# keras-team/keras-rs

Measured on AMD Instinct MI355X. Metric: embedding lookups/sec + DCN fwd+bwd step time, 26-table DLRM batch 65 536, higher is better.
Workload: dtype bf16; 1 GPU; C3 DLRM-small: 26 tables x 1000000 rows x 128 (bf16), global batch 65536, multi-hot ml_perf lengths (sum L = 214), uniform ids, DotInteraction(F=27) + 3 x FeatureCross(d=3456, projection=512), fused Adagrad on tables; global_batch=65536, parallelism=single GPU

## Files before the change

### include/krs.h

```cpp
#ifndef KRS_H_
#define KRS_H_

#include <stddef.h>
#include <stdint.h>

#ifdef __cplusplus
extern "C" {
#endif

#define KRS_VERSION 100

typedef enum krs_status {
  KRS_OK = 0,
  KRS_ERR_INVALID = -1,
  KRS_ERR_UNSUPPORTED = -2,
  KRS_ERR_LAUNCH = -3,
  KRS_ERR_WORKSPACE = -4
} krs_status;

typedef enum krs_dtype { KRS_F32 = 0, KRS_BF16 = 1, KRS_I8 = 2 } krs_dtype;
typedef enum krs_itype { KRS_I32 = 0, KRS_I64 = 1 } krs_itype;

typedef enum krs_combiner { KRS_SUM = 0, KRS_MEAN = 1, KRS_SQRTN = 2 } krs_combiner;

// ... 159 lines not shown
             void* workspace, size_t workspace_bytes, void* stream);
size_t krs_gemm_workspace_bytes(int64_t m, int64_t n, int64_t k, int a_is_km);

size_t krs_gemm_cross_bwd_workspace_bytes(int64_t m, int64_t n);
int krs_gemm_cross_bwd(const void* a, int64_t lda, const void* bt, int64_t ldb,
                       const void* r, int64_t ldr, float beta,
                       void* g_out, int64_t ldg,
                       const void* x0, const void* u, void* dz, void* dx0, int64_t ld, int dx0_accumulate,
                       const void* u_upper, int fold_direct, float* dbias, int64_t m, int64_t n, int64_t k, int act, int dtype,
                       void* workspace, size_t workspace_bytes, void* stream);
int krs_gemm_dense_bwd(const void* a, int64_t lda, const void* bt, int64_t ldb, void* g_out, int64_t ldg,
                       const void* y, void* dz, int64_t ld, float* dbias, int64_t m, int64_t n, int64_t k, int act,
                       int dtype, void* workspace, size_t workspace_bytes, void* stream);
enum { KRS_CROSS_BWD_NONE = 0, KRS_CROSS_BWD_TWO_CALL = 1, KRS_CROSS_BWD_PP64 = 2, KRS_CROSS_BWD_PP256 = 3 };
int krs_gemm_cross_bwd_last_route(int* epilogue);
int krs_gemm_cross_bwd_plan_route(const void* a, int64_t lda, const void* bt, int64_t ldb, const void* r, int64_t ldr,
                                  float beta, void* g_out, int64_t ldg, const void* x0, const void* u, void* dz, void* dx0,
                                  int64_t ld, int dx0_accumulate, const void* u_upper, int64_t m, int64_t n, int64_t k,
                                  int dtype, int* epilogue);

enum {
  KRS_GEMM_KERNEL_NONE = 0, KRS_GEMM_KERNEL_GENERIC = 1, KRS_GEMM_KERNEL_MFMA = 2, KRS_GEMM_KERNEL_GLDS = 3,
  KRS_GEMM_KERNEL_TN_GLDS = 4, KRS_GEMM_KERNEL_PP256 = 5, KRS_GEMM_KERNEL_PP256_KSTRIDED = 6, KRS_GEMM_KERNEL_PP64 = 7,
  KRS_GEMM_KERNEL_THIN = 8, KRS_GEMM_KERNEL_ROWDOT = 9, KRS_GEMM_KERNEL_SMALLK = 10
};
enum { KRS_GEMM_REDUCE_NONE = 0, KRS_GEMM_REDUCE_SCALAR = 1, KRS_GEMM_REDUCE_VEC4 = 2, KRS_GEMM_REDUCE_VEC8 = 3 };
typedef struct krs_gemm_route {
  int32_t kernel;
  int32_t splits;
  int32_t reduce;
  int32_t epilogue;
  int32_t ep_vec;
  int32_t thin_width;
  int32_t thin_is_a;
  int32_t schedule;
} krs_gemm_route;
enum { KRS_GEMM_SCHED_LDS_LANDING = 1, KRS_GEMM_SCHED_STAGGER = 2, KRS_GEMM_SCHED_X_IS_X0 = 4 };
int krs_gemm_last_route(krs_gemm_route* route);
int krs_gemm_plan_route(const void* a, int64_t lda, int a_is_km, const void* b, int64_t ldb, int b_is_nk, const void* c,
                        int64_t ldc, int64_t m, int64_t n, int64_t k, int in_dtype, int out_dtype,
                        const krs_gemm_epilogue* epilogue, size_t workspace_bytes, krs_gemm_route* route);

enum { KRS_GEMM_OPT_PIPELINE = 0, KRS_GEMM_OPT_EPI_SCHEDULE = 1 };
int krs_gemm_set_option(int key, int value);

enum { KRS_EMBED_OPT_PLAN = 2, KRS_EMBED_OPT_HOTROWS = 3, KRS_EMBED_OPT_RANK = 4, KRS_EMBED_OPT_APPLY_DEPTH = 5 };
int krs_embed_set_option(int key, int value);

size_t krs_colsum_workspace_bytes(int64_t m, int64_t n);
int krs_cross_epilogue_fwd(const void* u, const void* x0, const void* x, void* y,
                           int64_t m, int64_t n, int64_t ld, float diag_scale,
                           int dtype, void* stream);
// ... 237 lines not shown
```

### keras_rs_amd/_lib.py

```python

from __future__ import annotations

import ctypes as C
import os

import numpy as np
import torch

_HERE = os.path.dirname(os.path.abspath(__file__))
LIB_PATH = os.environ.get("KRS_LIB", os.path.join(_HERE, "libkrs_hip.so"))

F32, BF16, I8 = 0, 1, 2
I32, I64 = 0, 1
SUM, MEAN, SQRTN = 0, 1, 2
COMBINERS = {"sum": SUM, "mean": MEAN, "sqrtn": SQRTN}
ACT_NONE, ACT_RELU, ACT_SIGMOID, ACT_TANH = 0, 1, 2, 3
FLAG_ID_OUT_OF_RANGE = 1
FLAG_BAD_OFFSETS = 2
FLAG_CAPACITY_OVERFLOW = 4
FLAG_NONFINITE_ROW = 8
MAX_LIST = 4096

TABLE_DT = np.dtype(
    [("weights", "<u8"), ("slot", "<u8"), ("row_base", "<i8"), ("vocab", "<i4"), ("lr", "<f4")]
# ... 17 lines not shown
        ("ldx", C.c_int64),
        ("u_out", C.c_void_p),
        ("ldu", C.c_int64),
        ("r", C.c_void_p),
        ("ldr", C.c_int64),
        ("beta", C.c_float),
    ]


class GemmRoute(C.Structure):
    _fields_ = [(name, C.c_int32) for name in
                ("kernel", "splits", "reduce", "epilogue", "ep_vec", "thin_width", "thin_is_a", "schedule")]


GEMM_OPT_PIPELINE, GEMM_OPT_EPI_SCHEDULE = 0, 1
GEMM_SCHED_LDS_LANDING, GEMM_SCHED_STAGGER, GEMM_SCHED_X_IS_X0 = 1, 2, 4


class GemmQ8Route(C.Structure):
    _fields_ = [(name, C.c_int32) for name in ("kernel", "ep_vec", "k_tail", "epilogue")]


class EmbedFwdRoute(C.Structure):
    _fields_ = [(name, C.c_int32) for name in
                ("kernel", "lpr", "has_w", "stream", "hot_rows", "bpg", "table_dtype", "out_dtype")] + [("blocks", C.c_int64)]


class DotRoute(C.Structure):
    _fields_ = [(name, C.c_int32) for name in
                ("kernel", "dtype", "ks", "fr", "self", "multi", "acc", "ng", "lps_log2", "spw", "launches",
                 "lds_bytes")] + [("blocks", C.c_int64)]
# ... 18 lines not shown
    "krs_embed_bag_bwd_fused_sgd": (_I, _EMBED_BWD + [_P, _P]),
    "krs_embed_bag_bwd_fused_adagrad": (_I, _EMBED_BWD + [_P, _P]),
    "krs_embed_bag_bwd_fused_adagrad_rowwise": (_I, _EMBED_BWD + [_P, _P]),
    "krs_embed_bag_bwd_fused_adam": (_I, _EMBED_BWD + [_F, _F, _F, _F, _P, _P]),
    "krs_embed_bag_bwd_fused_ftrl": (_I, _EMBED_BWD + [_F, _F, _F, _F, _P, _P]),
    "krs_embed_bag_bwd_fused_adam_dyn": (_I, _EMBED_BWD + [_F, _F, _F, _P, _P, _P]),
    "krs_store_f32": (_I, [_P, _I64, _P, _I, _P]),
    "krs_embed_bag_bwd_sparse": (_I, [_P, _I, _P, _P, _P, _I, _I64, _I, _I, _I64, _P, _P, _P, _P, _P]),
    "krs_gemm": (_I, [_P, _I64, _I, _P, _I64, _I, _P, _I64, _I64, _I64, _I64, _I, _I, _P, _P, _SZ, _P]),
    "krs_gemm_workspace_bytes": (_SZ, [_I64, _I64, _I64, _I]),
    "krs_gemm_cross_bwd_workspace_bytes": (_SZ, [_I64, _I64]),
    "krs_gemm_cross_bwd": (_I, [_P, _I64, _P, _I64, _P, _I64, _F, _P, _I64, _P, _P, _P, _P, _I64, _I, _P, _I, _P,
                                _I64, _I64, _I64, _I, _I, _P, _SZ, _P]),
    "krs_gemm_dense_bwd": (_I, [_P, _I64, _P, _I64, _P, _I64, _P, _P, _I64, _P, _I64, _I64, _I64, _I, _I, _P, _SZ, _P]),
    "krs_gemm_cross_bwd_last_route": (_I, [_P]),
    "krs_gemm_cross_bwd_plan_route": (_I, [_P, _I64, _P, _I64, _P, _I64, _F, _P, _I64, _P, _P, _P, _P, _I64, _I, _P, _I64,
                                           _I64, _I64, _I, _P]),
    "krs_gemm_last_route": (_I, [_P]),
    "krs_gemm_plan_route": (_I, [_P, _I64, _I, _P, _I64, _I, _P, _I64, _I64, _I64, _I64, _I, _I, _P, _SZ, _P]),
    "krs_gemm_set_option": (_I, [_I, _I]),
    "krs_embed_set_option": (_I, [_I, _I]),
    "krs_colsum_workspace_bytes": (_SZ, [_I64, _I64]),
    "krs_cross_epilogue_fwd": (_I, [_P, _P, _P, _P, _I64, _I64, _I64, _F, _I, _P]),
    "krs_cross_epilogue_bwd": (_I, [_P, _P, _P, _P, _P, _P, _I, _P, _P, _I64, _I64, _I64, _F, _I, _I, _P, _SZ, _P]),
    "krs_cast_transpose": (_I, [_P, _I64, _I64, _I64, _I, _P, _I64, _P, _I64, _I, _P]),
    "krs_cast_transpose_many": (_I, [_I, _P, _P, _P, _I, _P, _P, _I, _P]),
    "krs_dense_act_bwd": (_I, [_P, _I64, _P, _I64, _P, _I64, _P, _I64, _I64, _I, _I, _P, _SZ, _P]),
    "krs_dense_adagrad": (_I, [_P, _P, _P, _P, _I, _F, _F, _P]),
    "krs_colsum": (_I, [_P, _I64, _I64, _I64, _I, _P, _P, _SZ, _P]),
    "krs_dot_interaction_fwd": (_I, [_P, _P, _I, _I64, _I, _I, _I, _I, _P, _I64, _P]),
# ... 162 lines not shown
```

### keras_rs_amd/csrc/gemm.hip

```cpp
#include <algorithm>
#include <cstdlib>
#include <cstring>

#include "gemm_device.h"
#include "gemm_plan.h"
#include "gemm_ring64.h"

namespace krs {
namespace {

constexpr int BM = gplan::kTile, BN = gplan::kTile;
constexpr int ROW_BYTES = gplan::kRowBytes;
constexpr int TILE_BYTES = gplan::kTileBytes;

template <int ES>
__device__ __forceinline__ void load_kstrided(const char* base, int64_t ld, int64_t row0, int64_t k0,
                                              int64_t rows, int64_t kk, u32x4 (&r)[4]) {
  constexpr int RPB = 16 / ES;
  constexpr int NRB = BM / RPB;
  const int t = threadIdx.x;
  const int rb = t % NRB;
  const int kb = t / NRB;
  const int64_t row = row0 + rb * RPB;
#pragma unroll
// ... 50 lines not shown
                                                          int64_t wm0, int64_t wn0, int split, EpiOperands (&o)[4],
                                                          const float* pre_bias = nullptr) {
  static_assert(NPFC == 2 || NPFC == 4, "two or four chunks of operands are fetched ahead");
  if constexpr (PREBIAS && NPFC == 4) {
#pragma unroll
    for (int c = 0; c < 4; ++c) epi_settle<EPI == 1>(o[c]);
  }
  epi_process<EPI, PREBIAS>(p, acc[0][0], o[0], stage, wm0, wn0, split, pre_bias);
  if constexpr (NPFC == 2) epi_prefetch<EPI>(p, o[2], wm0 + 64, wn0);
  epi_process<EPI, PREBIAS>(p, acc[0][1], o[1], stage, wm0 + 32, wn0, split, pre_bias);
  if constexpr (NPFC == 2) epi_prefetch<EPI>(p, o[3], wm0 + 96, wn0);
  epi_process<EPI, PREBIAS>(p, acc[1][0], o[2], stage, wm0 + 64, wn0, split, pre_bias);
  epi_process<EPI, PREBIAS>(p, acc[1][1], o[3], stage, wm0 + 96, wn0, split, pre_bias);
}

__device__ __forceinline__ void epi_land_issue(const GemmParams& p, uint32_t land, int64_t row0, int64_t wn0) {
  const int lane = threadIdx.x & 63;
  const int64_t gnc = min(wn0 + (lane & 7) * 8, p.n - 8);
  const uint16_t* src[8];
#pragma unroll
  for (int it = 0; it < 4; ++it) {
    const int64_t gmc = min(row0 + it * 8 + (lane >> 3), p.m - 1);
    src[it] = reinterpret_cast<const uint16_t*>(p.ep.x) + gmc * p.ep.ldx + gnc;
    src[4 + it] = reinterpret_cast<const uint16_t*>(p.ep.x0) + gmc * p.ep.ldx + gnc;
  }
#pragma unroll
  for (int i = 0; i < 8; ++i) {
    uint32_t keep;
    asm volatile("s_mov_b32 %0, m0\n\ts_mov_b32 m0, %2\n\ts_nop 0\n\tglobal_load_lds_dwordx4 %1, off nt\n\ts_mov_b32 m0, %0"
                 : "=&s"(keep)
                 : "v"(src[i]), "s"(land + i * 1024)
                 : "memory");
  }
}
template <int BEHIND>
__device__ __forceinline__ void epi_land_read(const char* land, EpiOperands& o) {
  static_assert(BEHIND >= 8 && BEHIND < 64, "vmcnt is a 6-bit counter");
  asm volatile("s_waitcnt vmcnt(%0)" ::"n"(BEHIND) : "memory");
  const int lane = threadIdx.x & 63;
#pragma unroll
  for (int it = 0; it < 4; ++it) {
    o.ex[it] = *reinterpret_cast<const uint4*>(land + it * 1024 + lane * 16);
    o.ex0[it] = *reinterpret_cast<const uint4*>(land + 4096 + it * 1024 + lane * 16);
  }
}
__device__ __forceinline__ void gemm_epilogue_wave128_land(const GemmParams& p, f32x16 (&acc)[2][2][2], float* stage, char* land,
                                                           int64_t wm0, int64_t wn0, int split, EpiOperands (&o)[4],
                                                           const float* pre_bias) {
// ... 385 lines not shown
        dz[q] = gx0 * act_grad_from_output(p.f_act, uv[q]);
        db[q] += dz[q];
        const float told = DX0 == 1 ? tv[q] : (DX0 == 2 ? rv[q] * tv[q] : 0.0f);
        tv[q] = __builtin_fmaf(g[q], uv[q], told);
        if (p.f_fold) tv[q] += g[q];
      }
      store8_bf16_nt(p.f_dz, gm * p.f_ld + gn, dz);
      if constexpr (DX0 != 3) store8_bf16_nt(p.f_dx0, gm * p.f_ld + gn, tv);
    }
    __builtin_amdgcn_fence(__ATOMIC_ACQ_REL, "wavefront");
    if (c < 3) {
      ld_x0u(c + 1, (c + 1) & 1);
      ld_rd(c + 1, (c + 1) & 1);
    }
  }
  if (p.f_partial) {
#pragma unroll
    for (int q = 0; q < 8; ++q) {
      float t = db[q];
      t += __shfl_xor(t, 8);
      t += __shfl_xor(t, 16);
      t += __shfl_xor(t, 32);
      db[q] = t;
    }
    if ((lane >> 3) == 0 && gn < p.n) {
      float* dst = p.f_partial + group * p.n + gn;
      *reinterpret_cast<float4*>(dst) = make_float4(db[0], db[1], db[2], db[3]);
      *reinterpret_cast<float4*>(dst + 4) = make_float4(db[4], db[5], db[6], db[7]);
    }
  }
// ... 255 lines not shown
  }
  if constexpr (NPFC > 0)
    gemm_epilogue_wave128_pre<EPI, NPFC>(p, acc, stage_f, m0 + wm * 128, n0 + wn * 64, split, opf);
  else
    gemm_epilogue_wave128<EPI>(p, acc, stage_f, m0 + wm * 128, n0 + wn * 64, split);
}

template <int EPI> constexpr int kRingEpiStreams = EPI == 1 ? 4 : EPI == kEpiCrossXIsX0 ? 3 : EPI == 2 ? 2 : 6;
template <int EPI, int SCHED>
__global__ __launch_bounds__(512) void gemm_pp64_kernel(const GemmParams p, int nt) {
  extern __shared__ __attribute__((aligned(16))) char smem[];
  constexpr int TM = 256, TN_ = 256;
  constexpr bool LAND = (SCHED & KRS_GEMM_SCHED_LDS_LANDING) != 0, STAGGER = (SCHED & KRS_GEMM_SCHED_STAGGER) != 0;
  static_assert(!LAND || EPI == 1, "only the cross build lands operands in LDS");
  static_assert(!STAGGER || EPI != 0, "the general build keeps the panel order");
  static_assert(gplan::kEpiStageBytes + gplan::kEpiLandBytes <= gplan::kRing64Lds, "the landing region lies inside the ring");
  const int lane = threadIdx.x & 63;
  const int wave = __builtin_amdgcn_readfirstlane(threadIdx.x >> 6);
  const int wm = wave >> 2, wn = wave & 3;
  const int64_t xcd = blockIdx.x & 7, slot_id = blockIdx.x >> 3;
  const int64_t tslot = slot_id / p.splits;
  const int split = (int)(slot_id - tslot * p.splits);
  const int64_t m_tile = (tslot / nt) * 8 + xcd;
  if (m_tile * TM >= p.m) return;
  const int64_t m0 = m_tile * TM, n0 = (STAGGER ? gplan::ring_tile_of_slot(tslot, nt, true).n_tile : tslot % nt) * TN_;
  const int64_t kbeg = (int64_t)split * p.k_per_split;
  const int64_t nb = (min(p.k, kbeg + p.k_per_split) - kbeg) / 64;
  if constexpr (STAGGER) {
    if (blockIdx.x < gplan::kCUs && (slot_id & 1)) {
      const uint64_t half_period = (uint64_t)nb * 78 + kRingEpiStreams<EPI> * 260, t0 = wall_clock64();
// ... 2 lines not shown
  }

  f32x16 acc[2][2][2];
#pragma unroll
  for (int h = 0; h < 2; ++h)
#pragma unroll
    for (int i = 0; i < 2; ++i)
#pragma unroll
      for (int j = 0; j < 2; ++j)
#pragma unroll
        for (int r = 0; r < 16; ++r) acc[h][i][j][r] = 0.0f;
  constexpr int NPFC = kRingEpiChunks<EPI>;
  EpiOperands opf[4];
  constexpr bool PREBIAS = LAND || EPI == kEpiCrossXIsX0;
  float pre_bias[8];
  ring64_main_loop<2, kRingEpiLoads<EPI> + (PREBIAS ? 2 : 0)>(smem, p, m0, n0, kbeg, nb, lane, wave, RingMmaBf16{acc}, [&]() {
    if constexpr (PREBIAS) epi_load_bias(p, n0 + wn * 64, pre_bias);
#pragma unroll
    for (int c = 0; c < NPFC; ++c) epi_prefetch<EPI>(p, opf[c], m0 + wm * 128 + c * 32, n0 + wn * 64);
  });
  float* stage_f = reinterpret_cast<float*>(smem) + wave * (32 * 68);
  if constexpr (EPI >= 3 && EPI <= 10) {
    gemm_epilogue_wave128_crossbwd<(EPI == 4 || EPI == 6) ? 1 : (EPI == 7 ? 2 : (EPI >= 8 ? 3 : 0)),
                                   EPI == 3 || EPI == 4 || EPI == 7, EPI < 9, EPI != 9>(
        p, acc, stage_f, m0 + wm * 128, n0 + wn * 64, (m0 >> 8) * 2 + wm);
    return;
  }
  if constexpr (LAND)
    gemm_epilogue_wave128_land(p, acc, stage_f, smem + gplan::kEpiStageBytes + wave * gplan::kEpiLandWaveBytes, m0 + wm * 128,
                               n0 + wn * 64, split, opf, pre_bias);
  else if constexpr (NPFC > 0)
    gemm_epilogue_wave128_pre<EPI, NPFC, PREBIAS>(p, acc, stage_f, m0 + wm * 128, n0 + wn * 64, split, opf, pre_bias);
  else
    gemm_epilogue_wave128<EPI>(p, acc, stage_f, m0 + wm * 128, n0 + wn * 64, split);
}

// ... 200 lines not shown
    acc = fmaf(av, bv, acc);
  }
  epilogue_store(p, i, j, acc);
}

int g_pipe = -1;
int gemm_pipe() {
  if (g_pipe < 0) {
    const char* e = getenv("KRS_GEMM_PIPE");
    g_pipe = e ? atoi(e) : 4;
    if (g_pipe != 0 && g_pipe != 5) g_pipe = 4;
  }
  return g_pipe;
}
constexpr int kEpiSchedDefault = 1;
int g_epi_sched = -1;
int gemm_epi_sched() {
  if (g_epi_sched < 0) {
    const char* e = getenv("KRS_GEMM_EPI_SCHEDULE");
    g_epi_sched = e ? atoi(e) : kEpiSchedDefault;
    if (g_epi_sched < 0 || g_epi_sched > 3) g_epi_sched = kEpiSchedDefault;
  }
  return g_epi_sched;
}

template <int First, int Last, class F>
int with_epilogue(int e, F&& f) {
  if constexpr (First < Last) {
    if (e != First) return with_epilogue<First + 1, Last>(e, f);
  }
// ... 166 lines not shown
                           workspace_bytes, true, call, pl);
  if (route) *route = pl.route;
  return rc;
}

extern "C" int krs_gemm_last_route(krs_gemm_route* route) {
  if (route) *route = g_route;
  return g_route.kernel;
}

extern "C" size_t krs_gemm_cross_bwd_workspace_bytes(int64_t m, int64_t n) {
  if (m <= 0 || n <= 0) return 0;
  return std::max(krs_colsum_workspace_bytes(m, n), (size_t)(2 * ceil_div(m, 256)) * (size_t)n * sizeof(float));
}

static thread_local int cb_route = KRS_CROSS_BWD_NONE, cb_epilogue = 0;

extern "C" int krs_gemm_cross_bwd_last_route(int* epilogue) {
  if (epilogue) *epilogue = cb_epilogue;
  return cb_route;
}

static int cross_bwd(const char* who, bool dense, const void* a, int64_t lda, const void* bt, int64_t ldb, const void* r,
                     int64_t ldr, float beta, void* g_out, int64_t ldg, const void* x0, const void* u, void* dz, void* dx0,
                     int64_t ld, int dx0_accumulate, const void* u_upper, int fold_direct, float* dbias, int64_t m,
                     int64_t n, int64_t k, int act, int dtype, void* workspace, size_t workspace_bytes, void* stream,
                     gplan::CrossBwdPlan* plan_only = nullptr) {
  const bool store_g = g_out != nullptr;
  if (dense && !g_out) { g_out = dz; ldg = ld; }
  if (!r) { ldr = n; beta = 0.0f; }
  KRS_REQUIRE(dtype == KRS_BF16 || dtype == KRS_F32, "%s: bad dtype", who);
  KRS_REQUIRE(m >= 0 && n >= 0 && k > 0 && ld >= n && ldg >= n && ldr >= n, "%s: bad sizes", who);
  krs_gemm_epilogue ep;
  memset(&ep, 0, sizeof(ep));
  ep.r = r; ep.ldr = ldr; ep.beta = beta;
  gplan::CrossBwdPlan cb;
  if (m > 0 && n > 0) {
    gplan::GemmCall call;
    if (int rc = gemm_plan(a, lda, 0, bt, ldb, 1, g_out, ldg, m, n, k, dtype, dtype, r ? &ep : nullptr, 0, false, call, cb.product))
      return rc;
    gplan::plan_cross_bwd(cb, r != nullptr, ld, al16(x0) && al16(u) && al16(dz) && al16(dx0) && al16(u_upper), dense, store_g,
                          dx0 != nullptr, dx0_accumulate != 0, u_upper != nullptr, gemm_epi_sched());
  }
  if (plan_only) { *plan_only = cb; return KRS_OK; }
  if (dbias) KRS_REQUIRE(workspace_bytes >= krs_gemm_cross_bwd_workspace_bytes(m, n) && (workspace || m == 0 || n == 0),
                         "%s: workspace too small (krs_gemm_cross_bwd_workspace_bytes)", who);
  hipStream_t st = reinterpret_cast<hipStream_t>(stream);
  if (m == 0 || n == 0) {
    if (dbias && n > 0) KRS_HIP(hipMemsetAsync(dbias, 0, (size_t)n * sizeof(float), st));
    return KRS_OK;
  }
  if (cb.route == KRS_CROSS_BWD_TWO_CALL) {
    cb_route = cb.route;
    if (int rc = gemm_run(a, lda, 0, bt, ldb, 1, g_out, ldg, m, n, k, dtype, dtype, r ? &ep : nullptr, nullptr, 0, stream,
                          false))
      return rc;
    KRS_REQUIRE(ldg == ld, "%s: the two-call form needs one row stride for G, x0, u, dz and dx0", who);
// ... 2 lines not shown
    if (u_upper) {
      KRS_REQUIRE(ldr == ld, "%s: the two-call form needs R on the common row stride", who);
      if (int rc = krs_cross_epilogue_bwd(r, u_upper, x0, x0, nullptr, dx0, 0, nullptr, nullptr, m, n, ld, 0.0f, KRS_ACT_NONE,
                                          dtype, nullptr, 0, stream)) return rc;
      dx0_accumulate = 1;
    }
    return krs_cross_epilogue_bwd(g_out, u, x0, x0, dz, dx0, dx0_accumulate, fold_direct ? dx0 : nullptr, dbias, m, n,
                                  ld, 0.0f, act, dtype, workspace, workspace_bytes, stream);
  }
  GemmParams p = gemm_params(a, lda, false, bt, ldb, true, g_out, ldg, m, n, k, KRS_BF16, &ep);
  p.ep_vec = 1;
  p.f_x0 = x0; p.f_u = u; p.f_uup = u_upper; p.f_dz = dz; p.f_dx0 = dx0; p.f_ld = ld; p.f_act = act; p.f_fold = fold_direct != 0;
  p.f_partial = dbias ? reinterpret_cast<float*>(workspace) : nullptr;
  const gplan::GemmPlan& pl = cb.product;
  const dim3 grid256((unsigned)pl.grid[0]), block((unsigned)pl.block);
  cb_route = cb.route; cb_epilogue = cb.epilogue;
  const int rc = with_epilogue<3, 10>(cb.epilogue, [&](auto E) {
    if (cb.route == KRS_CROSS_BWD_PP64)
      return cb.stagger ? launch_lds<gemm_pp64_kernel<E, KRS_GEMM_SCHED_STAGGER>>("gemm_pp64_kernel (fused cross backward)",
                                                                                  grid256, block, pl.lds, st, p, pl.nt)
                        : launch_lds<gemm_pp64_kernel<E, 0>>("gemm_pp64_kernel (fused cross backward)", grid256, block, pl.lds,
                                                             st, p, pl.nt);
    return launch_lds<gemm_pp256_kernel<false, 4, E>>("gemm_pp256_kernel (fused cross backward)", grid256, block, pl.lds, st,
                                                      p, 0, pl.nt);
  });
  if (rc != KRS_OK) return rc;
  return dbias ? finish_colsum(p.f_partial, 2 * ceil_div(m, 256), n, dbias, st) : KRS_OK;
}

extern "C" int krs_gemm_cross_bwd_plan_route(const void* a, int64_t lda, const void* bt, int64_t ldb, const void* r,
                                             int64_t ldr, float beta, void* g_out, int64_t ldg, const void* x0, const void* u,
                                             void* dz, void* dx0, int64_t ld, int dx0_accumulate, const void* u_upper,
                                             int64_t m, int64_t n, int64_t k, int dtype, int* epilogue) {
  gplan::CrossBwdPlan cb;
  const int rc = cross_bwd("krs_gemm_cross_bwd_plan_route", x0 == nullptr, a, lda, bt, ldb, r, ldr, beta, g_out, ldg, x0, u, dz,
                           dx0, ld, dx0_accumulate, u_upper, 0, nullptr, m, n, k, KRS_ACT_NONE, dtype, nullptr, 0, nullptr, &cb);
  if (epilogue) *epilogue = cb.epilogue;
  return rc ? rc : cb.route;
}

extern "C" int krs_gemm_cross_bwd(const void* a, int64_t lda, const void* bt, int64_t ldb, const void* r, int64_t ldr,
                                  float beta, void* g_out, int64_t ldg, const void* x0, const void* u, void* dz,
                                  void* dx0, int64_t ld, int dx0_accumulate, const void* u_upper, int fold_direct,
                                  float* dbias, int64_t m, int64_t n, int64_t k, int act, int dtype, void* workspace,
                                  size_t workspace_bytes, void* stream) {
  cb_route = KRS_CROSS_BWD_NONE; cb_epilogue = 0;
  KRS_REQUIRE((a && bt && x0 && u && dz && g_out) || m == 0 || n == 0, "krs_gemm_cross_bwd: null operand%s",
              x0 ? "" : " (x0 = NULL: the dense form is krs_gemm_dense_bwd)");
  KRS_REQUIRE(dx0 || (!r && !dx0_accumulate && !u_upper && !fold_direct),
              "krs_gemm_cross_bwd: dx0 = NULL (the term is left to the next launch's u_upper) is the form without R");
  KRS_REQUIRE(!u_upper || (r && !dx0_accumulate && beta == 1.0f),
              "krs_gemm_cross_bwd: u_upper (dx0 = R * u_upper + ...) needs R with beta = 1 and no dx0 to accumulate into");
  return cross_bwd("krs_gemm_cross_bwd", false, a, lda, bt, ldb, r, ldr, beta, g_out, ldg, x0, u, dz, dx0, ld,
                   dx0_accumulate, u_upper, fold_direct, dbias, m, n, k, act, dtype, workspace, workspace_bytes, stream);
}

extern "C" int krs_gemm_dense_bwd(const void* a, int64_t lda, const void* bt, int64_t ldb, void* g_out, int64_t ldg,
                                  const void* y, void* dz, int64_t ld, float* dbias, int64_t m, int64_t n, int64_t k,
                                  int act, int dtype, void* workspace, size_t workspace_bytes, void* stream) {
  cb_route = KRS_CROSS_BWD_NONE; cb_epilogue = 0;
  KRS_REQUIRE((a && bt && y && dz) || m == 0 || n == 0, "krs_gemm_dense_bwd: null operand");
  return cross_bwd("krs_gemm_dense_bwd", true, a, lda, bt, ldb, nullptr, n, 0.0f, g_out, ldg, nullptr, y, dz, nullptr, ld,
                   0, nullptr, 0, dbias, m, n, k, act, dtype, workspace, workspace_bytes, stream);
}
```

### keras_rs_amd/csrc/gemm_plan.h

```cpp
#ifndef KRS_GEMM_PLAN_H_
#define KRS_GEMM_PLAN_H_

#include <algorithm>
#include <cstddef>
#include <cstdint>

#include "../../include/krs.h"

namespace krs {

inline bool al16(const void* q) { return (reinterpret_cast<uintptr_t>(q) & 15) == 0; }

namespace gplan {

constexpr int kTile = 128, kRowBytes = 128;
constexpr int kLdsStride = kRowBytes + 16, kTileBytes = kTile * kLdsStride;
constexpr int kBigTile = 256, kCUs = 256;
constexpr int kFillTiles = 192;
constexpr int kRingBlock = 32, kRingDepth = 4;
constexpr int kRing64Block = 64, kRing64Depth = 3;
constexpr int kRingMinK = 256;
constexpr int kRingSplitMinK = 2048, kSplitMinK = 512;
constexpr int kGldsMinK = 1024;
constexpr int kThinMax = 16, kThinMinK = 1024, kThinMaxSplits = 128;
// ... 176 lines not shown
    p.grid[0] = cdiv(m, kSmallkRows);
    p.lds = (size_t)k * n * sizeof(float);
  } else {
    rt.kernel = KRS_GEMM_KERNEL_GENERIC;
    p.grid[0] = cdiv(m * n, 256);
  }
  if (rt.reduce) p.reduce_grid = cdiv(m * (rt.reduce == KRS_GEMM_REDUCE_VEC4 ? n / 4 : rt.reduce == KRS_GEMM_REDUCE_VEC8 ? n / 8 : n), 256);
  if (p.grid[0] * p.block > kMaxGridThreads || p.reduce_grid * 256 > kMaxGridThreads || p.grid[1] > kMaxGridYZ || p.grid[2] > kMaxGridYZ)
    return refuse(KRS_ERR_UNSUPPORTED, 0);
  return p;
}

struct CrossBwdPlan {
  int route = KRS_CROSS_BWD_NONE, epilogue = 0;
  bool stagger = false;
  GemmPlan product;
};

inline void plan_cross_bwd(CrossBwdPlan& cb, bool has_r, int64_t ld, bool al_streams, bool dense, bool store_g, bool has_dx0,
                           bool dx0_accumulate, bool has_u_upper, int epi_sched = 0) {
  const krs_gemm_route& rt = cb.product.route;
  cb.route = rt.kernel == KRS_GEMM_KERNEL_PP64 ? KRS_CROSS_BWD_PP64 : KRS_CROSS_BWD_PP256;
  cb.epilogue = 0;
  if ((rt.kernel != KRS_GEMM_KERNEL_PP64 && rt.kernel != KRS_GEMM_KERNEL_PP256) || rt.splits != 1 || !rt.ep_vec || ld % 8 != 0 ||
      !al_streams)
    cb.route = rt.kernel == KRS_GEMM_KERNEL_NONE ? KRS_CROSS_BWD_NONE : KRS_CROSS_BWD_TWO_CALL;
  else if (dense) cb.epilogue = store_g ? 10 : 9;
  else if (has_u_upper) cb.epilogue = 7;
  else if (has_r) cb.epilogue = dx0_accumulate ? 4 : 3;
  else cb.epilogue = !has_dx0 ? 8 : (dx0_accumulate ? 6 : 5);
  cb.stagger = cb.route == KRS_CROSS_BWD_PP64 && (epi_sched & 2);
}

}
}
#endif
```

### keras_rs_amd/dense_ops.py

```python

from __future__ import annotations

import ctypes as C
from typing import Sequence

import torch

from keras_rs_amd import _lib as L
from keras_rs_amd import probe

ACTS = {None: L.ACT_NONE, "linear": L.ACT_NONE, "relu": L.ACT_RELU, "sigmoid": L.ACT_SIGMOID,
        "tanh": L.ACT_TANH}


def gemm(a: torch.Tensor, b: torch.Tensor, *, a_is_km: bool = False, b_is_nk: bool = False,
         out_dtype: torch.dtype | None = None, bias: torch.Tensor | None = None, act: int = L.ACT_NONE,
         diag_scale: float = 0.0, x0: torch.Tensor | None = None, x: torch.Tensor | None = None,
         want_u: bool = False, r: torch.Tensor | None = None, beta: float = 1.0,
         out: torch.Tensor | None = None):
    a = L.rowmajor(a, "gemm A")
    b = L.rowmajor(b, "gemm B")
    if a.dtype != b.dtype:
        raise L.KrsError("gemm: A and B must share a dtype")
    m, k = (a.shape[1], a.shape[0]) if a_is_km else (a.shape[0], a.shape[1])
# ... 143 lines not shown
                                        L.ptr(dz), n, L.ptr(dbias), m, n, k, act, L.fdtype(a), L.ptr(ws), nbytes,
                                        L.stream_ptr())
    L.check(rc, "krs_gemm_dense_bwd")
    return dz, dbias, g


CROSS_BWD_ROUTES = {0: None, 1: "two_call", 2: "pp64", 3: "pp256"}


def last_cross_bwd_route():
    ep = C.c_int(0)
    route = int(L.lib().krs_gemm_cross_bwd_last_route(C.byref(ep)))
    return CROSS_BWD_ROUTES[route], int(ep.value)


GEMM_KERNELS = {0: None, 1: "generic", 2: "mfma", 3: "glds", 4: "tn_glds", 5: "pp256", 6: "pp256_kstrided", 7: "pp64",
                8: "thin", 9: "rowdot", 10: "smallk"}
GEMM_REDUCES = {0: None, 1: "scalar", 2: "vec4", 3: "vec8"}


def _route_dict(rt) -> dict:
    return dict(kernel=GEMM_KERNELS[rt.kernel], splits=int(rt.splits), reduce=GEMM_REDUCES[rt.reduce],
                epilogue=int(rt.epilogue), ep_vec=bool(rt.ep_vec), thin_width=int(rt.thin_width),
                thin_is_a=bool(rt.thin_is_a))


def last_gemm_route() -> dict:
    rt = L.GemmRoute()
    L.lib().krs_gemm_last_route(C.byref(rt))
    return _route_dict(rt)
# ... 321 lines not shown
```

Measured before the change: 1.506 billion lookups/s.

## Prefetch cross-backward epilogue operands one chunk ahead via LDS landing

Result: no change. 1.506 billion lookups/s (+0.0%).

```diff
diff --git a/include/krs.h b/include/krs.h
--- a/include/krs.h
+++ b/include/krs.h
@@ -197,6 +197,7 @@
                        int dtype, void* workspace, size_t workspace_bytes, void* stream);
 enum { KRS_CROSS_BWD_NONE = 0, KRS_CROSS_BWD_TWO_CALL = 1, KRS_CROSS_BWD_PP64 = 2, KRS_CROSS_BWD_PP256 = 3 };
 int krs_gemm_cross_bwd_last_route(int* epilogue);
+int krs_gemm_cross_bwd_last_schedule(void);
 int krs_gemm_cross_bwd_plan_route(const void* a, int64_t lda, const void* bt, int64_t ldb, const void* r, int64_t ldr,
                                   float beta, void* g_out, int64_t ldg, const void* x0, const void* u, void* dz, void* dx0,
                                   int64_t ld, int dx0_accumulate, const void* u_upper, int64_t m, int64_t n, int64_t k,
@@ -218,7 +219,7 @@
   int32_t thin_is_a;
   int32_t schedule;
 } krs_gemm_route;
-enum { KRS_GEMM_SCHED_LDS_LANDING = 1, KRS_GEMM_SCHED_STAGGER = 2, KRS_GEMM_SCHED_X_IS_X0 = 4 };
+enum { KRS_GEMM_SCHED_LDS_LANDING = 1, KRS_GEMM_SCHED_STAGGER = 2, KRS_GEMM_SCHED_X_IS_X0 = 4, KRS_GEMM_SCHED_BWD_AHEAD = 8 };
 int krs_gemm_last_route(krs_gemm_route* route);
 int krs_gemm_plan_route(const void* a, int64_t lda, int a_is_km, const void* b, int64_t ldb, int b_is_nk, const void* c,
                         int64_t ldc, int64_t m, int64_t n, int64_t k, int in_dtype, int out_dtype,
diff --git a/keras_rs_amd/_lib.py b/keras_rs_amd/_lib.py
--- a/keras_rs_amd/_lib.py
+++ b/keras_rs_amd/_lib.py
@@ -55,7 +55,7 @@
 
 
 GEMM_OPT_PIPELINE, GEMM_OPT_EPI_SCHEDULE = 0, 1
-GEMM_SCHED_LDS_LANDING, GEMM_SCHED_STAGGER, GEMM_SCHED_X_IS_X0 = 1, 2, 4
+GEMM_SCHED_LDS_LANDING, GEMM_SCHED_STAGGER, GEMM_SCHED_X_IS_X0, GEMM_SCHED_BWD_AHEAD = 1, 2, 4, 8
 
 
 class GemmQ8Route(C.Structure):
@@ -104,6 +104,7 @@
                                 _I64, _I64, _I64, _I, _I, _P, _SZ, _P]),
     "krs_gemm_dense_bwd": (_I, [_P, _I64, _P, _I64, _P, _I64, _P, _P, _I64, _P, _I64, _I64, _I64, _I, _I, _P, _SZ, _P]),
     "krs_gemm_cross_bwd_last_route": (_I, [_P]),
+    "krs_gemm_cross_bwd_last_schedule": (_I, []),
     "krs_gemm_cross_bwd_plan_route": (_I, [_P, _I64, _P, _I64, _P, _I64, _F, _P, _I64, _P, _P, _P, _P, _I64, _I, _P, _I64,
                                            _I64, _I64, _I, _P]),
     "krs_gemm_last_route": (_I, [_P]),
diff --git a/keras_rs_amd/csrc/gemm.hip b/keras_rs_amd/csrc/gemm.hip
--- a/keras_rs_amd/csrc/gemm.hip
+++ b/keras_rs_amd/csrc/gemm.hip
@@ -88,16 +88,7 @@
   epi_process<EPI, PREBIAS>(p, acc[1][1], o[3], stage, wm0 + 96, wn0, split, pre_bias);
 }
 
-__device__ __forceinline__ void epi_land_issue(const GemmParams& p, uint32_t land, int64_t row0, int64_t wn0) {
-  const int lane = threadIdx.x & 63;
-  const int64_t gnc = min(wn0 + (lane & 7) * 8, p.n - 8);
-  const uint16_t* src[8];
-#pragma unroll
-  for (int it = 0; it < 4; ++it) {
-    const int64_t gmc = min(row0 + it * 8 + (lane >> 3), p.m - 1);
-    src[it] = reinterpret_cast<const uint16_t*>(p.ep.x) + gmc * p.ep.ldx + gnc;
-    src[4 + it] = reinterpret_cast<const uint16_t*>(p.ep.x0) + gmc * p.ep.ldx + gnc;
-  }
+__device__ __forceinline__ void epi_land_dma8(uint32_t land, const uint16_t* const (&src)[8]) {
 #pragma unroll
   for (int i = 0; i < 8; ++i) {
     uint32_t keep;
@@ -106,6 +97,18 @@
                  : "v"(src[i]), "s"(land + i * 1024)
                  : "memory");
   }
+}
+__device__ __forceinline__ void epi_land_issue(const GemmParams& p, uint32_t land, int64_t row0, int64_t wn0) {
+  const int lane = threadIdx.x & 63;
+  const int64_t gnc = min(wn0 + (lane & 7) * 8, p.n - 8);
+  const uint16_t* src[8];
+#pragma unroll
+  for (int it = 0; it < 4; ++it) {
+    const int64_t gmc = min(row0 + it * 8 + (lane >> 3), p.m - 1);
+    src[it] = reinterpret_cast<const uint16_t*>(p.ep.x) + gmc * p.ep.ldx + gnc;
+    src[4 + it] = reinterpret_cast<const uint16_t*>(p.ep.x0) + gmc * p.ep.ldx + gnc;
+  }
+  epi_land_dma8(land, src);
 }
 template <int BEHIND>
 __device__ __forceinline__ void epi_land_read(const char* land, EpiOperands& o) {
@@ -521,6 +524,170 @@
       ld_rd(c + 1, (c + 1) & 1);
     }
   }
+  if (p.f_partial) {
+#pragma unroll
+    for (int q = 0; q < 8; ++q) {
+      float t = db[q];
+      t += __shfl_xor(t, 8);
+      t += __shfl_xor(t, 16);
+      t += __shfl_xor(t, 32);
+      db[q] = t;
+    }
+    if ((lane >> 3) == 0 && gn < p.n) {
+      float* dst = p.f_partial + group * p.n + gn;
+      *reinterpret_cast<float4*>(dst) = make_float4(db[0], db[1], db[2], db[3]);
+      *reinterpret_cast<float4*>(dst + 4) = make_float4(db[4], db[5], db[6], db[7]);
+    }
+  }
+}
+
+template <int DX0, bool HAS_R, bool X0, bool STORE_G>
+__device__ __forceinline__ void crossbwd_row(const GemmParams& p, const float* sv, int64_t gm, int64_t gn, const uint4& r8,
+                                             const uint4& x08, const uint4& u8, const uint4& d8, float (&db)[8]) {
+  float v[8], rv[8], x0v[8], uv[8], tv[8], g[8], dz[8];
+  const float4 v0 = *reinterpret_cast<const float4*>(sv);
+  const float4 v1 = *reinterpret_cast<const float4*>(sv + 4);
+  v[0] = v0.x; v[1] = v0.y; v[2] = v0.z; v[3] = v0.w; v[4] = v1.x; v[5] = v1.y; v[6] = v1.z; v[7] = v1.w;
+  if constexpr (HAS_R) {
+    unpack_bf16x8(r8, rv);
+#pragma unroll
+    for (int q = 0; q < 8; ++q) v[q] += p.ep.beta * rv[q];
+  }
+  const uint4 gq = make_uint4(pack_bf16x2(v[0], v[1]), pack_bf16x2(v[2], v[3]), pack_bf16x2(v[4], v[5]),
+                              pack_bf16x2(v[6], v[7]));
+  if constexpr (STORE_G) {
+    const u32x4 gs = {gq.x, gq.y, gq.z, gq.w};
+    __builtin_nontemporal_store(gs, reinterpret_cast<u32x4*>(reinterpret_cast<uint16_t*>(p.c) + gm * p.ldc + gn));
+  }
+  unpack_bf16x8(gq, g);
+  if constexpr (X0) unpack_bf16x8(x08, x0v);
+  unpack_bf16x8(u8, uv);
+  if constexpr (DX0 == 1 || DX0 == 2) unpack_bf16x8(d8, tv);
+  else {
+#pragma unroll
+    for (int q = 0; q < 8; ++q) tv[q] = 0.0f;
+  }
+#pragma unroll
+  for (int q = 0; q < 8; ++q) {
+    const float gx0 = X0 ? g[q] * x0v[q] : g[q];
+    dz[q] = gx0 * act_grad_from_output(p.f_act, uv[q]);
+    db[q] += dz[q];
+    const float told = DX0 == 1 ? tv[q] : (DX0 == 2 ? rv[q] * tv[q] : 0.0f);
+    tv[q] = __builtin_fmaf(g[q], uv[q], told);
+    if (p.f_fold) tv[q] += g[q];
+  }
+  store8_bf16_nt(p.f_dz, gm * p.f_ld + gn, dz);
+  if constexpr (DX0 != 3) store8_bf16_nt(p.f_dx0, gm * p.f_ld + gn, tv);
+}
+
+struct BwdAheadOperands {
+  uint4 x0[4], u[4];
+  uint4 r[2][4], d[2][4];
+};
+constexpr unsigned kBwdAheadBuilt = (1u << 3) | (1u << 5) | (1u << 8);
+template <int DX0, bool HAS_R> constexpr int kBwdAheadRdLoads = (HAS_R ? 4 : 0) + (DX0 == 1 || DX0 == 2 ? 4 : 0);
+template <int EPI> constexpr bool kBwdAheadRdTail = false;
+
+__device__ __forceinline__ void bwd_ahead_load_x0u(const GemmParams& p, BwdAheadOperands& o, int lane, int64_t row0,
+                                                   int64_t wn0) {
+  const int64_t gnc = min(wn0 + (lane & 7) * 8, p.n - 8);
+#pragma unroll
+  for (int it = 0; it < 4; ++it) {
+    const int64_t gmc = min(row0 + it * 8 + (lane >> 3), p.m - 1);
+    o.x0[it] = load8_bf16_nt(p.f_x0, gmc * p.f_ld + gnc);
+    o.u[it] = load8_bf16_nt(p.f_u, gmc * p.f_ld + gnc);
+  }
+}
+template <int DX0, bool HAS_R>
+__device__ __forceinline__ void bwd_ahead_load_rd(const GemmParams& p, BwdAheadOperands& o, int b, int lane, int64_t row0,
+                                                  int64_t wn0) {
+  const int64_t gnc = min(wn0 + (lane & 7) * 8, p.n - 8);
+#pragma unroll
+  for (int it = 0; it < 4; ++it) {
+    const int64_t gmc = min(row0 + it * 8 + (lane >> 3), p.m - 1);
+    if constexpr (HAS_R) o.r[b][it] = load8_bf16_nt(p.ep.r, gmc * p.ep.ldr + gnc);
+    if constexpr (DX0 == 1) o.d[b][it] = load8_bf16_nt(p.f_dx0, gmc * p.f_ld + gnc);
+    else if constexpr (DX0 == 2) o.d[b][it] = load8_bf16_nt(p.f_uup, gmc * p.f_ld + gnc);
+  }
+}
+__device__ __forceinline__ void bwd_ahead_land_issue(const GemmParams& p, uint32_t land, int lane, int64_t row0, int64_t wn0) {
+  const int64_t gnc = min(wn0 + (lane & 7) * 8, p.n - 8);
+  const uint16_t* src[8];
+#pragma unroll
+  for (int it = 0; it < 4; ++it) {
+    const int64_t gmc = min(row0 + it * 8 + (lane >> 3), p.m - 1);
+    src[it] = reinterpret_cast<const uint16_t*>(p.f_x0) + gmc * p.f_ld + gnc;
+    src[4 + it] = reinterpret_cast<const uint16_t*>(p.f_u) + gmc * p.f_ld + gnc;
+  }
+  asm volatile("s_waitcnt lgkmcnt(0)" ::: "memory");
+  epi_land_dma8(land, src);
+}
+template <int BEHIND>
+__device__ __forceinline__ void bwd_ahead_land_read(const char* land, BwdAheadOperands& o, int lane) {
+  static_assert(BEHIND >= 0 && BEHIND < 64, "vmcnt is a 6-bit counter");
+  asm volatile("s_waitcnt vmcnt(%0)" ::"n"(BEHIND) : "memory");
+#pragma unroll
+  for (int it = 0; it < 4; ++it) {
+    o.x0[it] = *reinterpret_cast<const uint4*>(land + it * 1024 + lane * 16);
+    o.u[it] = *reinterpret_cast<const uint4*>(land + 4096 + it * 1024 + lane * 16);
+  }
+}
+template <int DX0, bool HAS_R, bool RD_TAIL, bool INTERIOR>
+__device__ __forceinline__ void crossbwd_ahead_chunks(const GemmParams& p, f32x16 (&acc)[2][2][2], float* stage, const char* land,
+                                                      uint32_t land_lds, int64_t wm0, int64_t wn0, BwdAheadOperands& o,
+                                                      float (&db)[8]) {
+  constexpr int SST = 68, NRD = kBwdAheadRdLoads<DX0, HAS_R>, NST = INTERIOR ? 4 * (DX0 == 3 ? 2 : 3) : 0;
+  const int lane = threadIdx.x & 63;
+  const int frow = lane & 31, fhalf = lane >> 5;
+  const int ec = (lane & 7) * 8;
+  const int64_t gn = wn0 + ec;
+#pragma unroll
+  for (int c = 0; c < 4; ++c) {
+    const int64_t row0 = wm0 + c * 32;
+    const int b = c & 1;
+    f32x16(&acc2)[2] = acc[c >> 1][c & 1];
+#pragma unroll
+    for (int j = 0; j < 2; ++j)
+#pragma unroll
+      for (int r = 0; r < 16; ++r)
+        stage[((r & 3) + 8 * (r >> 2) + 4 * fhalf) * SST + j * 32 + frow] = acc2[j][r];
+    __builtin_amdgcn_fence(__ATOMIC_ACQ_REL, "wavefront");
+    if constexpr (!RD_TAIL) {
+      if (c == 0) bwd_ahead_load_rd<DX0, HAS_R>(p, o, 0, lane, row0, wn0);
+    }
+    if (c < 3) bwd_ahead_load_rd<DX0, HAS_R>(p, o, b ^ 1, lane, row0 + 32, wn0);
+    if (c == 1 || c == 2) bwd_ahead_land_read<NST + NRD>(land, o, lane);
+    if (c == 3) bwd_ahead_land_read<NST>(land, o, lane);
+    if (c < 3) bwd_ahead_land_issue(p, land_lds, lane, row0 + 32, wn0);
+#pragma unroll
+    for (int it = 0; it < 4; ++it) {
+      const int er_ = it * 8 + (lane >> 3);
+      const int64_t gm = row0 + er_;
+      if constexpr (!INTERIOR) {
+        if (gm >= p.m || gn >= p.n) continue;
+      }
+      crossbwd_row<DX0, HAS_R, true, true>(p, stage + er_ * SST + ec, gm, gn, o.r[b][it], o.x0[it], o.u[it], o.d[b][it], db);
+#pragma unroll
+      for (int q = 0; q < 8; ++q) asm volatile("" : "+v"(db[q]));
+      __builtin_amdgcn_sched_barrier(0);
+    }
+    __builtin_amdgcn_fence(__ATOMIC_ACQ_REL, "wavefront");
+  }
+}
+template <int DX0, bool HAS_R, bool RD_TAIL>
+__device__ __forceinline__ void gemm_epilogue_wave128_crossbwd_ahead(const GemmParams& p, f32x16 (&acc)[2][2][2], float* stage,
+                                                                     char* land, int64_t wm0, int64_t wn0, int64_t group,
+                                                                     BwdAheadOperands& o) {
+  const int lane = threadIdx.x & 63;
+  const int64_t gn = wn0 + (lane & 7) * 8;
+  const uint32_t land_lds = __builtin_amdgcn_readfirstlane((uint32_t)(uintptr_t)(__attribute__((address_space(3))) char*)land);
+  float db[8];
+#pragma unroll
+  for (int q = 0; q < 8; ++q) db[q] = 0.0f;
+  if (wm0 + 128 <= p.m && wn0 + 64 <= p.n)
+    crossbwd_ahead_chunks<DX0, HAS_R, RD_TAIL, true>(p, acc, stage, land, land_lds, wm0, wn0, o, db);
+  else
+    crossbwd_ahead_chunks<DX0, HAS_R, RD_TAIL, false>(p, acc, stage, land, land_lds, wm0, wn0, o, db);
   if (p.f_partial) {
 #pragma unroll
     for (int q = 0; q < 8; ++q) {
@@ -806,6 +973,8 @@
   constexpr bool LAND = (SCHED & KRS_GEMM_SCHED_LDS_LANDING) != 0, STAGGER = (SCHED & KRS_GEMM_SCHED_STAGGER) != 0;
   static_assert(!LAND || EPI == 1, "only the cross build lands operands in LDS");
   static_assert(!STAGGER || EPI != 0, "the general build keeps the panel order");
+  constexpr bool AHEAD = (SCHED & KRS_GEMM_SCHED_BWD_AHEAD) != 0;
+  static_assert(!AHEAD || ((kBwdAheadBuilt >> EPI) & 1u), "a fused backward build that requests a chunk ahead");
   static_assert(gplan::kEpiStageBytes + gplan::kEpiLandBytes <= gplan::kRing64Lds, "the landing region lies inside the ring");
   const int lane = threadIdx.x & 63;
   const int wave = __builtin_amdgcn_readfirstlane(threadIdx.x >> 6);
@@ -838,12 +1007,27 @@
   EpiOperands opf[4];
   constexpr bool PREBIAS = LAND || EPI == kEpiCrossXIsX0;
   float pre_bias[8];
-  ring64_main_loop<2, kRingEpiLoads<EPI> + (PREBIAS ? 2 : 0)>(smem, p, m0, n0, kbeg, nb, lane, wave, RingMmaBf16{acc}, [&]() {
-    if constexpr (PREBIAS) epi_load_bias(p, n0 + wn * 64, pre_bias);
-#pragma unroll
-    for (int c = 0; c < NPFC; ++c) epi_prefetch<EPI>(p, opf[c], m0 + wm * 128 + c * 32, n0 + wn * 64);
+  constexpr int BWD_DX0 = (EPI == 4 || EPI == 6) ? 1 : (EPI == 7 ? 2 : (EPI >= 8 ? 3 : 0));
+  constexpr bool BWD_R = EPI == 3 || EPI == 4 || EPI == 7, BWD_RD_TAIL = AHEAD && kBwdAheadRdTail<EPI>;
+  constexpr int NPF = AHEAD ? 8 + (BWD_RD_TAIL ? kBwdAheadRdLoads<BWD_DX0, BWD_R> : 0) : kRingEpiLoads<EPI> + (PREBIAS ? 2 : 0);
+  BwdAheadOperands bo;
+  ring64_main_loop<2, NPF>(smem, p, m0, n0, kbeg, nb, lane, wave, RingMmaBf16{acc}, [&]() {
+    if constexpr (AHEAD) {
+      bwd_ahead_load_x0u(p, bo, lane, m0 + wm * 128, n0 + wn * 64);
+      if constexpr (BWD_RD_TAIL) bwd_ahead_load_rd<BWD_DX0, BWD_R>(p, bo, 0, lane, m0 + wm * 128, n0 + wn * 64);
+    } else {
+      if constexpr (PREBIAS) epi_load_bias(p, n0 + wn * 64, pre_bias);
+#pragma unroll
+      for (int c = 0; c < NPFC; ++c) epi_prefetch<EPI>(p, opf[c], m0 + wm * 128 + c * 32, n0 + wn * 64);
+    }
   });
   float* stage_f = reinterpret_cast<float*>(smem) + wave * (32 * 68);
+  if constexpr (AHEAD) {
+    gemm_epilogue_wave128_crossbwd_ahead<BWD_DX0, BWD_R, BWD_RD_TAIL>(
+        p, acc, stage_f, smem + gplan::kEpiStageBytes + wave * gplan::kEpiLandWaveBytes, m0 + wm * 128, n0 + wn * 64,
+        (m0 >> 8) * 2 + wm, bo);
+    return;
+  }
   if constexpr (EPI >= 3 && EPI <= 10) {
     gemm_epilogue_wave128_crossbwd<(EPI == 4 || EPI == 6) ? 1 : (EPI == 7 ? 2 : (EPI >= 8 ? 3 : 0)),
                                    EPI == 3 || EPI == 4 || EPI == 7, EPI < 9, EPI != 9>(
@@ -1074,6 +1258,8 @@
   return g_pipe;
 }
 constexpr int kEpiSchedDefault = 1;
+constexpr unsigned kBwdAheadBuilds = kBwdAheadBuilt;
+static_assert((kBwdAheadBuilds & ~kBwdAheadBuilt) == 0, "a build ships the schedule only where it exists");
 int g_epi_sched = -1;
 int gemm_epi_sched() {
   if (g_epi_sched < 0) {
@@ -1270,12 +1456,14 @@
   return std::max(krs_colsum_workspace_bytes(m, n), (size_t)(2 * ceil_div(m, 256)) * (size_t)n * sizeof(float));
 }
 
-static thread_local int cb_route = KRS_CROSS_BWD_NONE, cb_epilogue = 0;
+static thread_local int cb_route = KRS_CROSS_BWD_NONE, cb_epilogue = 0, cb_schedule = 0;
 
 extern "C" int krs_gemm_cross_bwd_last_route(int* epilogue) {
   if (epilogue) *epilogue = cb_epilogue;
   return cb_route;
 }
+
+extern "C" int krs_gemm_cross_bwd_last_schedule(void) { return cb_schedule; }
 
 static int cross_bwd(const char* who, bool dense, const void* a, int64_t lda, const void* bt, int64_t ldb, const void* r,
                      int64_t ldr, float beta, void* g_out, int64_t ldg, const void* x0, const void* u, void* dz, void* dx0,
@@ -1296,7 +1484,7 @@
     if (int rc = gemm_plan(a, lda, 0, bt, ldb, 1, g_out, ldg, m, n, k, dtype, dtype, r ? &ep : nullptr, 0, false, call, cb.product))
       return rc;
     gplan::plan_cross_bwd(cb, r != nullptr, ld, al16(x0) && al16(u) && al16(dz) && al16(dx0) && al16(u_upper), dense, store_g,
-                          dx0 != nullptr, dx0_accumulate != 0, u_upper != nullptr, gemm_epi_sched());
+                          dx0 != nullptr, dx0_accumulate != 0, u_upper != nullptr, gemm_epi_sched(), kBwdAheadBuilds);
   }
   if (plan_only) { *plan_only = cb; return KRS_OK; }
   if (dbias) KRS_REQUIRE(workspace_bytes >= krs_gemm_cross_bwd_workspace_bytes(m, n) && (workspace || m == 0 || n == 0),
@@ -1329,8 +1517,16 @@
   p.f_partial = dbias ? reinterpret_cast<float*>(workspace) : nullptr;
   const gplan::GemmPlan& pl = cb.product;
   const dim3 grid256((unsigned)pl.grid[0]), block((unsigned)pl.block);
-  cb_route = cb.route; cb_epilogue = cb.epilogue;
+  cb_route = cb.route; cb_epilogue = cb.epilogue; cb_schedule = cb.schedule;
   const int rc = with_epilogue<3, 10>(cb.epilogue, [&](auto E) {
+    if constexpr ((kBwdAheadBuilt >> E) & 1u) {
+      constexpr int AHEAD = KRS_GEMM_SCHED_BWD_AHEAD;
+      if (cb.schedule & AHEAD)
+        return cb.stagger ? launch_lds<gemm_pp64_kernel<E, AHEAD | KRS_GEMM_SCHED_STAGGER>>(
+                                "gemm_pp64_kernel (fused cross backward)", grid256, block, pl.lds, st, p, pl.nt)
+                          : launch_lds<gemm_pp64_kernel<E, AHEAD>>("gemm_pp64_kernel (fused cross backward)", grid256, block,
+                                                                   pl.lds, st, p, pl.nt);
+    }
     if (cb.route == KRS_CROSS_BWD_PP64)
       return cb.stagger ? launch_lds<gemm_pp64_kernel<E, KRS_GEMM_SCHED_STAGGER>>("gemm_pp64_kernel (fused cross backward)",
                                                                                   grid256, block, pl.lds, st, p, pl.nt)
@@ -1359,7 +1555,7 @@
                                   void* dx0, int64_t ld, int dx0_accumulate, const void* u_upper, int fold_direct,
                                   float* dbias, int64_t m, int64_t n, int64_t k, int act, int dtype, void* workspace,
                                   size_t workspace_bytes, void* stream) {
-  cb_route = KRS_CROSS_BWD_NONE; cb_epilogue = 0;
+  cb_route = KRS_CROSS_BWD_NONE; cb_epilogue = 0; cb_schedule = 0;
   KRS_REQUIRE((a && bt && x0 && u && dz && g_out) || m == 0 || n == 0, "krs_gemm_cross_bwd: null operand%s",
               x0 ? "" : " (x0 = NULL: the dense form is krs_gemm_dense_bwd)");
   KRS_REQUIRE(dx0 || (!r && !dx0_accumulate && !u_upper && !fold_direct),
@@ -1373,7 +1569,7 @@
 extern "C" int krs_gemm_dense_bwd(const void* a, int64_t lda, const void* bt, int64_t ldb, void* g_out, int64_t ldg,
                                   const void* y, void* dz, int64_t ld, float* dbias, int64_t m, int64_t n, int64_t k,
                                   int act, int dtype, void* workspace, size_t workspace_bytes, void* stream) {
-  cb_route = KRS_CROSS_BWD_NONE; cb_epilogue = 0;
+  cb_route = KRS_CROSS_BWD_NONE; cb_epilogue = 0; cb_schedule = 0;
   KRS_REQUIRE((a && bt && y && dz) || m == 0 || n == 0, "krs_gemm_dense_bwd: null operand");
   return cross_bwd("krs_gemm_dense_bwd", true, a, lda, bt, ldb, nullptr, n, 0.0f, g_out, ldg, nullptr, y, dz, nullptr, ld,
                    0, nullptr, 0, dbias, m, n, k, act, dtype, workspace, workspace_bytes, stream);
diff --git a/keras_rs_amd/csrc/gemm_plan.h b/keras_rs_amd/csrc/gemm_plan.h
--- a/keras_rs_amd/csrc/gemm_plan.h
+++ b/keras_rs_amd/csrc/gemm_plan.h
@@ -214,11 +214,12 @@
 struct CrossBwdPlan {
   int route = KRS_CROSS_BWD_NONE, epilogue = 0;
   bool stagger = false;
+  int schedule = 0;
   GemmPlan product;
 };
 
 inline void plan_cross_bwd(CrossBwdPlan& cb, bool has_r, int64_t ld, bool al_streams, bool dense, bool store_g, bool has_dx0,
-                           bool dx0_accumulate, bool has_u_upper, int epi_sched = 0) {
+                           bool dx0_accumulate, bool has_u_upper, int epi_sched = 0, unsigned ahead_builds = 0) {
   const krs_gemm_route& rt = cb.product.route;
   cb.route = rt.kernel == KRS_GEMM_KERNEL_PP64 ? KRS_CROSS_BWD_PP64 : KRS_CROSS_BWD_PP256;
   cb.epilogue = 0;
@@ -230,6 +231,11 @@
   else if (has_r) cb.epilogue = dx0_accumulate ? 4 : 3;
   else cb.epilogue = !has_dx0 ? 8 : (dx0_accumulate ? 6 : 5);
   cb.stagger = cb.route == KRS_CROSS_BWD_PP64 && (epi_sched & 2);
+  cb.schedule = 0;
+  if (cb.route == KRS_CROSS_BWD_PP64 && cb.epilogue >= 3 && cb.epilogue <= 8) {
+    if (cb.stagger) cb.schedule |= KRS_GEMM_SCHED_STAGGER;
+    if ((epi_sched & 1) && ((ahead_builds >> cb.epilogue) & 1u)) cb.schedule |= KRS_GEMM_SCHED_BWD_AHEAD;
+  }
 }
 
 }
diff --git a/keras_rs_amd/dense_ops.py b/keras_rs_amd/dense_ops.py
--- a/keras_rs_amd/dense_ops.py
+++ b/keras_rs_amd/dense_ops.py
@@ -181,6 +181,12 @@
     return CROSS_BWD_ROUTES[route], int(ep.value)
 
 
+def last_cross_bwd_schedule() -> frozenset:
+    bits = int(L.lib().krs_gemm_cross_bwd_last_schedule())
+    names = ((L.GEMM_SCHED_STAGGER, "stagger"), (L.GEMM_SCHED_BWD_AHEAD, "bwd_ahead"))
+    return frozenset(name for bit, name in names if bits & bit)
+
+
 GEMM_KERNELS = {0: None, 1: "generic", 2: "mfma", 3: "glds", 4: "tn_glds", 5: "pp256", 6: "pp256_kstrided", 7: "pp64",
                 8: "thin", 9: "rowdot", 10: "smallk"}
 GEMM_REDUCES = {0: None, 1: "scalar", 2: "vec4", 3: "vec8"}
```
